# YIVEK/aom-av1-lavish

Measured on AMD Instinct MI355X. Metric: superblocks/s (fwd_txfm+quant+SAD RDO inner loop), 1080p cpu-used=6, 1/2/4/8 GPU, higher is better.
Workload: dtype int32; 1 GPU; rdo: 1920x1080 8-bit frame per step; C2 fwd_txfm2d + quantize_fp (qindex 128) of all 14 TX sizes <=32x32 x every valid TX type + C3 DIAMOND full-pel search of every 16x16 block x 7 refs (downsampled SAD, MV_COST_ENTROPY default nmv context, sadperbit 4, errorperbit 31, cost list, step_param 0; candidate rows from the references' tiled copy, rebuilt per step); 510 SB64/frame; parallelism=frame-per-rank x1, legs=C3 on a second stream beside C2 (C3 in at most 384 workgroups)

## Files before the change

### aom-av1-lavish_amd/csrc/txq.hip

```cpp
#include <atomic>

#include "txq_dev.h"

namespace lavish {

template <int LS>
__device__ __forceinline__ int32_t quant_rt(int32_t c, bool ac, int kind, int highbd,
                                            const QP& qp) {
  if (kind == LAVISH_QUANT_FP)
    return highbd ? quant_one<LS, LAVISH_QUANT_FP, true>(c, ac, qp)
                  : quant_one<LS, LAVISH_QUANT_FP, false>(c, ac, qp);
  return highbd ? quant_one<LS, LAVISH_QUANT_B, true>(c, ac, qp)
                : quant_one<LS, LAVISH_QUANT_B, false>(c, ac, qp);
}

constexpr int kFrameStreams = 3;
constexpr int kFanDefault = 3;

template <int W, int H>
__global__ __launch_bounds__(256, 2) void txq_plane_kernel(TxqArgs a) {
  __shared__ __attribute__((aligned(16))) char lds[TxqLds<W, H>::kBytes];
  txq_plane_body<W, H>(a, blockIdx.x, lds);
}

template <int CLS>
__global__ __launch_bounds__(256, 2) void txq_multi_kernel(TxqDispatch d, TxqArgs a0, TxqArgs a1,
                                                           TxqArgs a2, TxqArgs a3, TxqArgs a4,
                                                           TxqArgs a5, TxqArgs a6, TxqArgs a7,
                                                           TxqArgs a8) {
  __shared__ __attribute__((aligned(16))) char lds[class_lds(CLS)];
  txq_multi_body<CLS>(d, a0, a1, a2, a3, a4, a5, a6, a7, a8, blockIdx.x, lds);
}

template <int LS>
__global__ __launch_bounds__(256) void quant_kernel(const int32_t* coeff, int n,
                                                     const int16_t* scan, int kind,
                                                     int highbd, QP qp,
                                                     int32_t* qcoeff, int32_t* dqcoeff,
                                                     uint16_t* eob) {
  __shared__ int red[4];
  const size_t base = (size_t)blockIdx.x * n;
  const int tid = threadIdx.x;
  int last = 0;
  for (int i = tid; i < n; i += 256) {
    const int rc = scan[i];
    const int32_t c = coeff[base + rc];
    const int32_t q = quant_rt<LS>(c, rc != 0, kind, highbd, qp);
    qcoeff[base + rc] = q;
    const int32_t cs = c >> 31, m = (q ^ cs) - cs;
    const int32_t d = rc != 0 ? qp.dequant[1] : qp.dequant[0];
    const int32_t dm = (int32_t)((uint32_t)m * (uint32_t)d) >> LS;
    dqcoeff[base + rc] = (dm ^ cs) - cs;
    if (q != 0) last = max(last, i + 1);
  }
#pragma unroll
  for (int m = 1; m < 64; m <<= 1) last = max(last, __shfl_xor(last, m));
  if ((tid & 63) == 0) red[tid >> 6] = last;
  __syncthreads();
  if (tid == 0) eob[blockIdx.x] = (uint16_t)max(max(red[0], red[1]), max(red[2], red[3]));
}

static void build_chunks(TxqArgs& a, int nbg) {
  int cnt = 0, sz[16] = {}, ti[16][16];
  for (int vk = 0; vk < 4; ++vk) {
    int n = 0;
    for (int i = 0; i < a.ntypes; ++i)
      if (((kVtxPacked >> (2 * a.types[i])) & 3) == (uint32_t)vk) ti[cnt][n++] = i;
    if (n) sz[cnt++] = n;
  }
  while (nbg * cnt < 2048 && cnt < 16) {
    int big = 0;
    for (int g = 1; g < cnt; ++g)
      if (sz[g] > sz[big]) big = g;
    if (sz[big] < 2) break;
    const int keep = (sz[big] + 1) / 2;
    for (int i = keep; i < sz[big]; ++i) ti[cnt][i - keep] = ti[big][i];
    sz[cnt++] = sz[big] - keep;
    sz[big] = keep;
  }
  int o = 0;
  for (int g = 0; g < cnt; ++g) {
    a.chunk_off[g] = o;
    for (int i = 0; i < sz[g]; ++i) a.chunk_ti[o++] = ti[g][i];
  }
  a.chunk_off[cnt] = o;
  a.tgroups = cnt;
}

template <int W, int H>
static int plan_plane(TxqArgs& a) {
  constexpr int P = Tile<W, H>::P * 4;
  const int nbg = (a.nblocks + P - 1) / P;
  if (nbg == 0) return 0;
  build_chunks(a, nbg);
  return ((nbg + 7) / 8) * 8 * a.tgroups;
}

template <int W, int H>
static void launch_plane(TxqArgs a, hipStream_t s) {
  const int grid = plan_plane<W, H>(a);
  if (grid == 0) return;
  hipLaunchKernelGGL((txq_plane_kernel<W, H>), dim3(grid), dim3(256), 0, s, a);
  LAVISH_CHECK(hipGetLastError());
}

static int plan_size(int tx_size, TxqArgs& a) {
  switch (tx_size) {
    case 0: return plan_plane<4, 4>(a);
    case 1: return plan_plane<8, 8>(a);
    case 2: return plan_plane<16, 16>(a);
    case 3: return plan_plane<32, 32>(a);
    case 5: return plan_plane<4, 8>(a);
    case 6: return plan_plane<8, 4>(a);
    case 7: return plan_plane<8, 16>(a);
    case 8: return plan_plane<16, 8>(a);
    case 9: return plan_plane<16, 32>(a);
    case 10: return plan_plane<32, 16>(a);
    case 13: return plan_plane<4, 16>(a);
    case 14: return plan_plane<16, 4>(a);
    case 15: return plan_plane<8, 32>(a);
    case 16: return plan_plane<32, 8>(a);
    default: return -1;
  }
}

static QP to_qp(const LavishQuantParams* p) {
  QP q{};
  if (p) {
    for (int i = 0; i < 2; ++i) {
      q.zbin[i] = p->zbin[i];
      q.round[i] = p->round[i];
      q.quant[i] = p->quant[i];
      q.quant_shift[i] = p->quant_shift[i];
      q.dequant[i] = p->dequant[i];
    }
  }
  return q;
}

int txq_args(const int16_t* residual, int stride, int width, int height, int tx_size,
             uint32_t type_mask, int bd, int quant_kind, const LavishQuantParams* qp,
             int32_t* qcoeff, int32_t* dqcoeff, uint16_t* eob, int32_t* coeff, TxqArgs& a);

int txq_plane(const int16_t* residual, int stride, int width, int height, int tx_size,
              uint32_t type_mask, int bd, int quant_kind, const LavishQuantParams* qp,
              int32_t* qcoeff, int32_t* dqcoeff, uint16_t* eob, int32_t* coeff,
              hipStream_t s) {
  if (tx_size < 0 || tx_size >= 19) return -1;
  const int W = tx_w(tx_size), H = tx_h(tx_size);
  if (quant_kind < 0 || quant_kind > 2) return -3;
  if (quant_kind != LAVISH_QUANT_NONE && qp == nullptr) return -3;
  if (quant_kind == LAVISH_QUANT_FP && !quant_fp_params_ok(qp)) return kErrQuantParams;
  if (width <= 0 || height <= 0 || stride < width) return -4;
  if (W > 32 || H > 32)
    return txq_plane_64(residual, stride, width, height, tx_size, type_mask, bd, quant_kind, qp,
                        qcoeff, dqcoeff, eob, coeff, s);
  TxqArgs a{};
  const int rc = txq_args(residual, stride, width, height, tx_size, type_mask, bd, quant_kind,
                          qp, qcoeff, dqcoeff, eob, coeff, a);
  if (rc) return rc;
  switch (tx_size) {
    case 0: launch_plane<4, 4>(a, s); break;
    case 1: launch_plane<8, 8>(a, s); break;
    case 2: launch_plane<16, 16>(a, s); break;
    case 3: launch_plane<32, 32>(a, s); break;
    case 5: launch_plane<4, 8>(a, s); break;
    case 6: launch_plane<8, 4>(a, s); break;
    case 7: launch_plane<8, 16>(a, s); break;
    case 8: launch_plane<16, 8>(a, s); break;
    case 9: launch_plane<16, 32>(a, s); break;
    case 10: launch_plane<32, 16>(a, s); break;
    case 13: launch_plane<4, 16>(a, s); break;
    case 14: launch_plane<16, 4>(a, s); break;
    case 15: launch_plane<8, 32>(a, s); break;
    case 16: launch_plane<32, 8>(a, s); break;
    default: return -2;
  }
  return 0;
}

int txq_args(const int16_t* residual, int stride, int width, int height, int tx_size,
             uint32_t type_mask, int bd, int quant_kind, const LavishQuantParams* qp,
             int32_t* qcoeff, int32_t* dqcoeff, uint16_t* eob, int32_t* coeff, TxqArgs& a) {
  const int W = tx_w(tx_size), H = tx_h(tx_size);
// ... 30 lines not shown
    case 0:
      hipLaunchKernelGGL(quant_kernel<0>, dim3(nblocks), dim3(256), 0, s, coeff, n, scan,
                         quant_kind, hb, q, qcoeff, dqcoeff, eob);
      break;
    case 1:
      hipLaunchKernelGGL(quant_kernel<1>, dim3(nblocks), dim3(256), 0, s, coeff, n, scan,
                         quant_kind, hb, q, qcoeff, dqcoeff, eob);
      break;
    case 2:
      hipLaunchKernelGGL(quant_kernel<2>, dim3(nblocks), dim3(256), 0, s, coeff, n, scan,
                         quant_kind, hb, q, qcoeff, dqcoeff, eob);
      break;
    default:
      return -2;
  }
  LAVISH_CHECK(hipGetLastError());
  return 0;
}

struct FrameStreams {
  int device = -1;
  hipStream_t s[kFrameStreams] = {};
  hipEvent_t fork = nullptr, join[kFrameStreams] = {};
};
static thread_local FrameStreams t_fs;
struct FanSet {
  FrameStreams fs;
};
static thread_local FanSet* t_fan_own = nullptr;

static void frame_streams_init(FrameStreams& f, int dev) {
  for (int i = 1; i < kFrameStreams; ++i) {
    LAVISH_CHECK(hipStreamCreateWithFlags(&f.s[i], hipStreamNonBlocking));
    LAVISH_CHECK(hipEventCreateWithFlags(&f.join[i], hipEventDisableTiming));
  }
  LAVISH_CHECK(hipEventCreateWithFlags(&f.fork, hipEventDisableTiming));
  f.device = dev;
}

static FrameStreams& frame_streams() {
  if (t_fan_own != nullptr) return t_fan_own->fs;
  int dev = 0;
  LAVISH_CHECK(hipGetDevice(&dev));
  if (t_fs.device != dev) frame_streams_init(t_fs, dev);
  return t_fs;
}

FanSet* fan_create() {
  int dev = 0;
  LAVISH_CHECK(hipGetDevice(&dev));
  FanSet* f = new FanSet();
  frame_streams_init(f->fs, dev);
  return f;
}

void fan_destroy(FanSet* f) {
  if (f == nullptr) return;
  if (t_fan_own == f) t_fan_own = nullptr;
  for (int i = 1; i < kFrameStreams; ++i) {
    LAVISH_CHECK(hipStreamDestroy(f->fs.s[i]));
    LAVISH_CHECK(hipEventDestroy(f->fs.join[i]));
  }
  LAVISH_CHECK(hipEventDestroy(f->fs.fork));
  delete f;
}

void fan_use(FanSet* f) { t_fan_own = f; }

static std::atomic<int> g_fan_width{kFanDefault};
int fan_width() { return g_fan_width.load(std::memory_order_relaxed); }
int set_fan_width(int w) {
  if (w < 1 || w > kFrameStreams) return -1;
  g_fan_width.store(w, std::memory_order_relaxed);
  return 0;
}

hipStream_t* fan_out(hipStream_t caller) {
  FrameStreams& fs = frame_streams();
  fs.s[0] = caller;
  LAVISH_CHECK(hipEventRecord(fs.fork, caller));
  for (int i = 1; i < kFrameStreams; ++i) LAVISH_CHECK(hipStreamWaitEvent(fs.s[i], fs.fork, 0));
  return fs.s;
}

void fan_in(hipStream_t caller) {
  FrameStreams& fs = frame_streams();
  for (int i = 1; i < kFrameStreams; ++i) {
    LAVISH_CHECK(hipEventRecord(fs.join[i], fs.s[i]));
    LAVISH_CHECK(hipStreamWaitEvent(caller, fs.join[i], 0));
  }
}

int txq_frame_plan(const int16_t* residual, int stride, int width, int height, uint32_t size_mask,
                   const uint32_t* type_masks, int bd, int quant_kind, const LavishQuantParams* qp,
                   int32_t* const* qcoeff, int32_t* const* dqcoeff, uint16_t* const* eob, int cls,
                   TxqMulti& m, int& grid) {
  if (quant_kind == LAVISH_QUANT_FP && qp != nullptr && !quant_fp_params_ok(qp))
    return kErrQuantParams;
  int order[19], n = 0;
  for (int s = 0; s < 19; ++s)
    if (((size_mask >> s) & 1) && tx_w(s) <= 32 && tx_h(s) <= 32 && (txq_class(s) ? 1 : 0) == cls)
      order[n++] = s;
  auto work = [&](int s) {
    return (long)__builtin_popcount(type_masks[s]) * max_eob(s) * (width / tx_w(s)) *
           (height / tx_h(s));
  };
  for (int i = 1; i < n; ++i)
    for (int j = i; j > 0 && work(order[j]) > work(order[j - 1]); --j) {
      const int t = order[j];
      order[j] = order[j - 1];
      order[j - 1] = t;
    }
  m = TxqMulti{};
  int g = 0;
  for (int i = 0; i < n; ++i) {
    const int s = order[i];
    if (m.d.n == kMultiMax) return -2;
    TxqArgs& a = m.a[txq_slot(s)];
    const int rc = txq_args(residual, stride, width, height, s, type_masks[s], bd, quant_kind, qp,
                            qcoeff[s], dqcoeff[s], eob[s], nullptr, a);
    if (rc) return rc;
    const int sg = plan_size(s, a);
    if (sg <= 0) continue;
    m.d.code[m.d.n] = s;
    m.d.wg0[m.d.n] = g;
    g += sg;
    ++m.d.n;
  }
  m.d.wg0[m.d.n] = g;
  grid = g;
  return 0;
}

int txq_frame(const int16_t* residual, int stride, int width, int height, uint32_t size_mask,
              const uint32_t* type_masks, int bd, int quant_kind, const LavishQuantParams* qp,
              int32_t* const* qcoeff, int32_t* const* dqcoeff, uint16_t* const* eob,
              hipStream_t caller) {
  if (quant_kind == LAVISH_QUANT_FP && qp != nullptr && !quant_fp_params_ok(qp))
    return kErrQuantParams;
  for (int s = 0; s < 19; ++s) {
    if (!((size_mask >> s) & 1) || (tx_w(s) <= 32 && tx_h(s) <= 32)) continue;
    const int rc = txq_plane(residual, stride, width, height, s, type_masks[s], bd, quant_kind,
                             qp, qcoeff[s], dqcoeff[s], eob[s], nullptr, caller);
    if (rc) return rc;
  }
  for (int cls = 1; cls >= 0; --cls) {
    TxqMulti m;
    int g = 0;
    const int rc = txq_frame_plan(residual, stride, width, height, size_mask, type_masks, bd,
                                  quant_kind, qp, qcoeff, dqcoeff, eob, cls, m, g);
    if (rc) return rc;
    if (g == 0) continue;
    if (cls == 0)
      hipLaunchKernelGGL(txq_multi_kernel<0>, dim3(g), dim3(256), 0, caller, m.d, m.a[0], m.a[1],
                         m.a[2], m.a[3], m.a[4], m.a[5], m.a[6], m.a[7], m.a[8]);
    else
      hipLaunchKernelGGL(txq_multi_kernel<1>, dim3(g), dim3(256), 0, caller, m.d, m.a[0], m.a[1],
                         m.a[2], m.a[3], m.a[4], m.a[5], m.a[6], m.a[7], m.a[8]);
    LAVISH_CHECK(hipGetLastError());
  }
  return 0;
}

}

extern "C" int lavish_set_fan_width(int streams) { return lavish::set_fan_width(streams); }

extern "C" int lavish_txq_frame(const int16_t* residual, int stride, int width, int height,
                                uint32_t size_mask, const uint32_t* type_masks, int bit_depth,
                                int quant_kind, const LavishQuantParams* qp,
                                int32_t* const* qcoeff, int32_t* const* dqcoeff,
                                uint16_t* const* eob, void* stream) {
  return lavish::txq_frame(residual, stride, width, height, size_mask, type_masks, bit_depth,
                           quant_kind, qp, qcoeff, dqcoeff, eob, (hipStream_t)stream);
}

extern "C" int lavish_txq_plane(const int16_t* residual, int stride, int width, int height,
                                int tx_size, uint32_t type_mask, int bit_depth,
                                int quant_kind, const LavishQuantParams* qp,
                                int32_t* qcoeff, int32_t* dqcoeff, uint16_t* eob,
                                int32_t* coeff, void* stream) {
  return lavish::txq_plane(residual, stride, width, height, tx_size, type_mask, bit_depth,
                           quant_kind, qp, qcoeff, dqcoeff, eob, coeff,
                           (hipStream_t)stream);
}

extern "C" int lavish_quantize_batch(const int32_t* coeff, int n, int nblocks,
                                     const int16_t* scan, const int16_t* iscan,
                                     int log_scale, int bit_depth, int quant_kind,
                                     const LavishQuantParams* qp, int32_t* qcoeff,
                                     int32_t* dqcoeff, uint16_t* eob, void* stream) {
  (void)iscan;
  return lavish::quantize_batch(coeff, n, nblocks, scan, log_scale, bit_depth, quant_kind,
                                qp, qcoeff, dqcoeff, eob, (hipStream_t)stream);
}
```

### aom-av1-lavish_amd/csrc/txq_dev.h

```cpp
#pragma once

#include "lane_red.h"
#include "lavish_internal.h"
#include "quant_dev.h"

namespace lavish {

struct TxqArgs {
  const int16_t* res;
  int stride;
  int bw;
  int nblocks;
  int ntypes;
  int types[16];
  int tgroups;
  int chunk_off[17];
  int chunk_ti[16];
  int quant_kind;
  int highbd;
  QP qp;
  const int16_t* iscan_default;
  int32_t* qcoeff;
  int32_t* dqcoeff;
  uint16_t* eob;
  int32_t* coeff;
};

template <int W, int H>
struct Tile {
  static constexpr int MN = W < H ? W : H;
  static constexpr int P = 64 / MN;
  static constexpr int CPT = W / MN;
  static constexpr int RPT = H / MN;
  static constexpr int N = W * H;
  static constexpr int T1S = W + 1;
  static constexpr int T1 = P * H * T1S;
  static constexpr int T2 = P * N;
};

template <int W, int H, bool FAST, int QK, bool HBD>
__device__ __forceinline__ void txq_types(const TxqArgs& a,
                                          const int32_t (&res)[Tile<W, H>::CPT][H],
                                          int32_t* t1, int32_t* t2, const int16_t* isc, int lane,
                                          int blk0, int nvalid, int c0, int c1) {
  using C = TxCfg<W, H>;
  using T = Tile<W, H>;
  constexpr int N = T::N, T1S = T::T1S;
  constexpr int LS = C::log_scale;
  {
    const int t = __builtin_amdgcn_readfirstlane(a.types[a.chunk_ti[c0]]);
    const int vt = (kVtxPacked >> (2 * t)) & 3;
    const int kc = vt == 3 ? 2 : (vt == 0 ? 0 : 1);
    const bool ud = vt == 2;
#pragma unroll
    for (int k = 0; k < T::CPT; ++k) {
      const int j = k * 64 + lane;
      const int b = j / W, c = j % W;
      int32_t in[H], out[H];
#pragma unroll
      for (int r = 0; r < H; ++r) {
        const int32_t x = ud ? res[k][H - 1 - r] : res[k][r];
        if constexpr (FAST) in[r] = x * (1 << C::s0);
        else in[r] = round_shift_1<-C::s0>(x);
      }
      fwd_1d<H, C::cos_bit_col, FAST>(kc, in, out);
#pragma unroll
      for (int r = 0; r < H; ++r) t1[(b * H + r) * T1S + c] = round_shift_1<-C::s1>(out[r]);
    }
    wave_sync();
  }

  int qf_rnd[2], qf_thr1[2], qf_qt[2];
#pragma unroll
  for (int i = 0; i < 2; ++i) {
    qf_rnd[i] = (a.qp.round[i] + ((1 << LS) >> 1)) >> LS;
    qf_qt[i] = a.qp.quant[i];
    qf_thr1[i] = ((a.qp.dequant[i] + (1 << (1 + LS)) - 1) >> (1 + LS)) - 1;
  }

  for (int ci = c0; ci < c1; ++ci) {
    const int ti = __builtin_amdgcn_readfirstlane(a.chunk_ti[ci]);
    const int t = __builtin_amdgcn_readfirstlane(a.types[ti]);
    const int ht = (kHtxPacked >> (2 * t)) & 3;
    const int kr = ht == 3 ? 2 : (ht == 0 ? 0 : 1);
    const bool lr = ht == 2;
    const int skind = t < 10 ? 0 : ((t & 1) ? 1 : 2);

#pragma unroll
    for (int k = 0; k < T::RPT; ++k) {
      const int j = k * 64 + lane;
      const int b = j / H, r = j % H;
      int32_t in[W], out[W];
      const int32_t* row = t1 + (b * H + r) * T1S;
      if (lr) {
#pragma unroll
        for (int c = 0; c < W; ++c) in[c] = row[W - 1 - c];
      } else {
#pragma unroll
        for (int c = 0; c < W; ++c) in[c] = row[c];
      }
      fwd_1d<W, C::cos_bit_row, FAST>(kr, in, out);
      const size_t obase = ((size_t)ti * a.nblocks + blk0 + b) * N;
      const int16_t* iscan = isc + skind * N;
      int last = 0;
      if constexpr (QK == LAVISH_QUANT_FP && FAST && !HBD) {
        const bool dcl = r == 0;
        const int rnd0 = dcl ? qf_rnd[0] : qf_rnd[1];
        const int qt0 = dcl ? qf_qt[0] : qf_qt[1];
        const int thr0 = dcl ? qf_thr1[0] : qf_thr1[1];
#pragma unroll
        for (int c = 0; c < W; ++c) {
          int32_t v = round_shift_1<-C::s2>(out[c]);
          if constexpr (C::rect2) v = rshift64((int64_t)v * 5793, 12);
          const int rc = c * H + r;
          if (a.coeff != nullptr) {
            if (b < nvalid) a.coeff[obase + rc] = v;
          }
          const int32_t sgn = v >> 31;
          const int32_t av = (v ^ sgn) - sgn;
          const int32_t pass = ((c ? qf_thr1[1] : thr0) - av) >> 31;
          const int32_t t = min(av + (c ? qf_rnd[1] : rnd0), 32767);
          const int32_t qa = (mul_i24(t, c ? qf_qt[1] : qt0) >> (16 - LS)) & pass;
          const int32_t q = (qa ^ sgn) - sgn;
          t2[b * N + rc] = q;
          const int32_t nz = (qa + 0x7FFFFF) >> 23;
          last = max(last, ((int)iscan[rc] + 1) & -nz);
        }
      } else {
#pragma unroll
      for (int c = 0; c < W; ++c) {
        int32_t v = round_shift_1<-C::s2>(out[c]);
        if constexpr (C::rect2) v = rshift64((int64_t)v * 5793, 12);
        const int rc = c * H + r;
        int32_t q = 0;
        if constexpr (QK == LAVISH_QUANT_NONE) {
          if (b < nvalid) a.coeff[obase + rc] = v;
        } else {
          if (a.coeff != nullptr) {
            if (b < nvalid) a.coeff[obase + rc] = v;
          }
          q = quant_one<LS, QK, HBD, FAST>(v, c != 0 || r != 0, a.qp);
        }
        t2[b * N + rc] = q;
        const int pos1 = iscan[rc] + 1;
        last = q != 0 ? max(last, pos1) : last;
      }
      }
      last = lane_max<H>(last);
      if (r == 0 && b < nvalid && a.eob != nullptr)
        a.eob[(size_t)ti * a.nblocks + blk0 + b] = (uint16_t)last;
    }
    wave_sync();

    if (a.qcoeff != nullptr) {
      const int total = nvalid * N;
      const size_t gbase = ((size_t)ti * a.nblocks + blk0) * N;
      for (int i = lane * 4; i < total; i += 64 * 4) {
        const v4i q4 = *reinterpret_cast<const v4i*>(&t2[i]);
        __builtin_nontemporal_store(q4, reinterpret_cast<v4i*>(&a.qcoeff[gbase + i]));
        if (a.dqcoeff != nullptr) {
          const int rc0 = i % N;
          v4i d4;
          d4.x = dequant_one<LS, FAST>(q4.x, rc0 != 0, a.qp);
          d4.y = dequant_one<LS, FAST>(q4.y, 1, a.qp);
          d4.z = dequant_one<LS, FAST>(q4.z, 1, a.qp);
          d4.w = dequant_one<LS, FAST>(q4.w, 1, a.qp);
          __builtin_nontemporal_store(d4, reinterpret_cast<v4i*>(&a.dqcoeff[gbase + i]));
        }
      }
    }
    wave_sync();
  }
}

template <int W, int H>
struct TxqLds {
  using T = Tile<W, H>;
  static constexpr int kT2Off = (4 * T::T1 * 4 + 15) & ~15;
  static constexpr int kIscOff = kT2Off + 4 * T::T2 * 4;
  static constexpr int kBytes = kIscOff + 3 * T::N * 2;
};

template <int W, int H>
__device__ __forceinline__ void txq_plane_body(const TxqArgs& a, int id, char* lds) {
  using T = Tile<W, H>;
  using LL = TxqLds<W, H>;
  constexpr int H_ = H;
  int32_t* t1s = reinterpret_cast<int32_t*>(lds);
  int32_t* t2s = reinterpret_cast<int32_t*>(lds + LL::kT2Off);
  int16_t* isc = reinterpret_cast<int16_t*>(lds + LL::kIscOff);

  const int inner = id & 7, rest = id >> 3;
  const int tg = rest % a.tgroups, quad = (rest / a.tgroups) * 8 + inner;
  const int ntiles = (a.nblocks + T::P - 1) / T::P;
  if (quad * 4 >= ntiles) return;
  const int c0 = a.chunk_off[tg], c1 = a.chunk_off[tg + 1];

  const int tid = threadIdx.x;
  for (int i = tid; i < T::N; i += 256) {
    isc[i] = a.iscan_default[i];
    isc[T::N + i] = (int16_t)i;
    isc[2 * T::N + i] = (int16_t)((i % H) * W + i / H);
  }
  __syncthreads();

  const int wave = tid >> 6, lane = tid & 63;
  const int tile = quad * 4 + wave;
  if (tile >= ntiles) return;
  const int blk0 = tile * T::P;
  const int nvalid = min(T::P, a.nblocks - blk0);
  int32_t* t1 = t1s + wave * T::T1;
  int32_t* t2 = t2s + wave * T::T2;

  int32_t res[T::CPT][H_];
  int32_t amax = 0;
#pragma unroll
  for (int k = 0; k < T::CPT; ++k) {
    const int j = k * 64 + lane;
    const int b = j / W, c = j % W;
    const int blk = blk0 + b;
    if (b < nvalid) {
      const int by = blk / a.bw, bx = blk - by * a.bw;
      const int16_t* src = a.res + (size_t)by * H * a.stride + bx * W + c;
#pragma unroll
      for (int r = 0; r < H; ++r) {
        res[k][r] = src[(size_t)r * a.stride];
        amax = max(amax, abs(res[k][r]));
      }
    } else {
#pragma unroll
      for (int r = 0; r < H; ++r) res[k][r] = 0;
    }
  }
  const bool fast = __builtin_amdgcn_ballot_w64(amax > kFastResidualMax) == 0;
#define LAVISH_TXQ_RUN(F, Q, HB) \
  txq_types<W, H, F, Q, HB>(a, res, t1, t2, isc, lane, blk0, nvalid, c0, c1)
  const int qk = a.quant_kind;
  if (qk == LAVISH_QUANT_NONE) {
    if (fast) LAVISH_TXQ_RUN(true, LAVISH_QUANT_NONE, false);
    else LAVISH_TXQ_RUN(false, LAVISH_QUANT_NONE, false);
  } else if (qk == LAVISH_QUANT_FP) {
    if (a.highbd) {
      if (fast) LAVISH_TXQ_RUN(true, LAVISH_QUANT_FP, true);
      else LAVISH_TXQ_RUN(false, LAVISH_QUANT_FP, true);
    } else {
      if (fast) LAVISH_TXQ_RUN(true, LAVISH_QUANT_FP, false);
      else LAVISH_TXQ_RUN(false, LAVISH_QUANT_FP, false);
    }
  } else {
    if (a.highbd) {
      if (fast) LAVISH_TXQ_RUN(true, LAVISH_QUANT_B, true);
      else LAVISH_TXQ_RUN(false, LAVISH_QUANT_B, true);
    } else {
      if (fast) LAVISH_TXQ_RUN(true, LAVISH_QUANT_B, false);
      else LAVISH_TXQ_RUN(false, LAVISH_QUANT_B, false);
    }
  }
#undef LAVISH_TXQ_RUN
}

constexpr int kMultiMax = 9;
struct TxqDispatch {
  int code[kMultiMax];
  int wg0[kMultiMax + 1];
  int n;
};
struct TxqMulti {
  TxqArgs a[kMultiMax];
  TxqDispatch d;
};
__host__ __device__ constexpr int txq_slot(int s) {
  return s == 0 ? 0 : s == 1 ? 1 : s == 2 ? 2 : s == 5 ? 3 : s == 6 ? 4 : s == 7 ? 5
       : s == 8 ? 6 : s == 13 ? 7 : s == 14 ? 8
       : s == 3 ? 0 : s == 9 ? 1 : s == 10 ? 2 : s == 15 ? 3 : s == 16 ? 4 : -1;
}
static_assert(sizeof(TxqMulti) <= 4096, "kernel argument size");

constexpr int lds_bytes(int s) {
  return s == 0 ? TxqLds<4, 4>::kBytes : s == 1 ? TxqLds<8, 8>::kBytes
       : s == 2 ? TxqLds<16, 16>::kBytes : s == 3 ? TxqLds<32, 32>::kBytes
       : s == 5 ? TxqLds<4, 8>::kBytes : s == 6 ? TxqLds<8, 4>::kBytes
       : s == 7 ? TxqLds<8, 16>::kBytes : s == 8 ? TxqLds<16, 8>::kBytes
       : s == 9 ? TxqLds<16, 32>::kBytes : s == 10 ? TxqLds<32, 16>::kBytes
       : s == 13 ? TxqLds<4, 16>::kBytes : s == 14 ? TxqLds<16, 4>::kBytes
       : s == 15 ? TxqLds<8, 32>::kBytes : s == 16 ? TxqLds<32, 8>::kBytes : 0;
}
__host__ __device__ constexpr bool txq_class(int s) {
  return s == 3 || s == 9 || s == 10 || s == 15 || s == 16;
}
constexpr int class_lds(int cls) {
  int m = 16;
  for (int s = 0; s < 17; ++s)
    if ((s < 4 || s > 4) && s != 11 && s != 12 && lds_bytes(s) > 0 && (txq_class(s) ? 1 : 0) == cls)
      m = lds_bytes(s) > m ? lds_bytes(s) : m;
  return m;
}

template <int CLS>
__device__ __forceinline__ void txq_multi_body(const TxqDispatch& d, const TxqArgs& a0,
                                               const TxqArgs& a1, const TxqArgs& a2,
                                               const TxqArgs& a3, const TxqArgs& a4,
                                               const TxqArgs& a5, const TxqArgs& a6,
                                               const TxqArgs& a7, const TxqArgs& a8, int g,
                                               char* lds) {
  int code = d.code[0], id = g;
#pragma unroll
  for (int k = 1; k < kMultiMax; ++k) {
    if (k < d.n && g >= d.wg0[k]) {
      code = d.code[k];
      id = g - d.wg0[k];
    }
  }
  if constexpr (CLS == 0) {
    switch (code) {
      case 0: txq_plane_body<4, 4>(a0, id, lds); break;
      case 1: txq_plane_body<8, 8>(a1, id, lds); break;
      case 2: txq_plane_body<16, 16>(a2, id, lds); break;
      case 5: txq_plane_body<4, 8>(a3, id, lds); break;
      case 6: txq_plane_body<8, 4>(a4, id, lds); break;
      case 7: txq_plane_body<8, 16>(a5, id, lds); break;
      case 8: txq_plane_body<16, 8>(a6, id, lds); break;
      case 13: txq_plane_body<4, 16>(a7, id, lds); break;
      case 14: txq_plane_body<16, 4>(a8, id, lds); break;
      default: break;
    }
  } else {
    switch (code) {
      case 3: txq_plane_body<32, 32>(a0, id, lds); break;
      case 9: txq_plane_body<16, 32>(a1, id, lds); break;
      case 10: txq_plane_body<32, 16>(a2, id, lds); break;
      case 15: txq_plane_body<8, 32>(a3, id, lds); break;
      case 16: txq_plane_body<32, 8>(a4, id, lds); break;
      default: break;
    }
  }
}

int txq_frame_plan(const int16_t* residual, int stride, int width, int height, uint32_t size_mask,
                   const uint32_t* type_masks, int bd, int quant_kind, const LavishQuantParams* qp,
                   int32_t* const* qcoeff, int32_t* const* dqcoeff, uint16_t* const* eob, int cls,
                   TxqMulti& m, int& grid);

int txq_frame(const int16_t* residual, int stride, int width, int height, uint32_t size_mask,
              const uint32_t* type_masks, int bd, int quant_kind, const LavishQuantParams* qp,
              int32_t* const* qcoeff, int32_t* const* dqcoeff, uint16_t* const* eob,
              hipStream_t caller);

}
```

### aom-av1-lavish_amd/lavish_dsp/__init__.py

```python
import ctypes
import os

import numpy as np

_HERE = os.path.dirname(os.path.abspath(__file__))
LIB_PATH = os.environ.get("LAVISH_HIP_LIB") or os.path.join(os.path.dirname(_HERE),
                                                            "liblavish_hip.so")

if not os.path.exists(LIB_PATH):
    raise ImportError(
        "liblavish_hip.so not found at %s -- build it with `make -C aom-av1-lavish_amd` "
        "(or __graft_entry__.build()); there is no CPU fallback" % LIB_PATH)

try:
    import torch
except ImportError:
    pass

_lib = ctypes.CDLL(LIB_PATH)

TX_SIZES = ["4x4", "8x8", "16x16", "32x32", "64x64", "4x8", "8x4", "8x16", "16x8",
            "16x32", "32x16", "32x64", "64x32", "4x16", "16x4", "8x32", "32x8", "16x64",
            "64x16"]
TX_W = [4, 8, 16, 32, 64, 4, 8, 8, 16, 16, 32, 32, 64, 4, 16, 8, 32, 16, 64]
# ... 4 lines not shown
QUANT_FP, QUANT_B, QUANT_NONE = 0, 1, 2


def max_eob(tx_size):
    if tx_size in (17, 18):
        return 512
    if TX_W[tx_size] == 64 or TX_H[tx_size] == 64:
        return 1024
    return TX_W[tx_size] * TX_H[tx_size]


def tx_scale(tx_size):
    p = TX_W[tx_size] * TX_H[tx_size]
    return int(p > 256) + int(p > 1024)


def tx_type_valid(tx_size, tx_type):
    m = max(TX_W[tx_size], TX_H[tx_size])
    if m == 64:
        return tx_type == 0
    if m == 32:
        return tx_type in (0, 9)
    return 0 <= tx_type < 16


def valid_type_mask(tx_size):
    return sum(1 << t for t in range(16) if tx_type_valid(tx_size, t))


class TxfmParam(ctypes.Structure):
    _fields_ = [("tx_type", ctypes.c_uint8), ("tx_size", ctypes.c_uint8),
                ("lossless", ctypes.c_int), ("bd", ctypes.c_int), ("is_hbd", ctypes.c_int),
                ("tx_set_type", ctypes.c_uint8), ("eob", ctypes.c_int)]


class QuantParams(ctypes.Structure):
    _fields_ = [(n, ctypes.c_int16 * 2) for n in
                ("zbin", "round", "quant", "quant_shift", "dequant")]

    def as_dict(self):
        return {n: np.array(list(getattr(self, n)), np.int16) for n, _ in self._fields_}


_vp, _i32, _i64 = ctypes.c_void_p, ctypes.c_int, ctypes.c_int64
_lib.lavish_hip_status.restype = _i32
_lib.lavish_hip_status_string.restype = ctypes.c_char_p
_lib.lavish_hip_set_abort_on_error.argtypes = [_i32]
_lib.lavish_hip_init.argtypes = [_i32]
_lib.lavish_hip_version.restype = _i32
_lib.lavish_build_quant_params.argtypes = [_i32, _i32, _i32, _i32, _i32,
                                           ctypes.POINTER(QuantParams)]
_lib.lavish_scan.restype = ctypes.POINTER(ctypes.c_int16)
_lib.lavish_scan.argtypes = [_i32, _i32]
_lib.lavish_iscan.restype = ctypes.POINTER(ctypes.c_int16)
_lib.lavish_iscan.argtypes = [_i32, _i32]
_lib.lavish_txq_plane.argtypes = [_vp, _i32, _i32, _i32, _i32, ctypes.c_uint32, _i32, _i32,
                                  ctypes.POINTER(QuantParams), _vp, _vp, _vp, _vp, _vp]
_lib.lavish_txq_plane.restype = _i32
_lib.lavish_txq_frame.argtypes = [_vp, _i32, _i32, _i32, ctypes.c_uint32, _vp, _i32, _i32,
                                  ctypes.POINTER(QuantParams), _vp, _vp, _vp, _vp]
_lib.lavish_txq_frame.restype = _i32
_lib.lavish_quantize_batch.argtypes = [_vp, _i32, _i32, _vp, _vp, _i32, _i32, _i32,
                                       ctypes.POINTER(QuantParams), _vp, _vp, _vp, _vp]
_lib.lavish_quantize_batch.restype = _i32

_FWD2D = {}
for _s, _name in enumerate(TX_SIZES):
    f = getattr(_lib, "av1_fwd_txfm2d_%s_hip" % _name)
    f.argtypes = [_vp, _vp, _i32, ctypes.c_uint8, _i32]
    f.restype = None
    _FWD2D[_s] = f
_lib.av1_lowbd_fwd_txfm_hip.argtypes = [_vp, _vp, _i32, ctypes.POINTER(TxfmParam)]


class PlaneQuant(ctypes.Structure):
    _fields_ = [(n, ctypes.c_int16 * 2) for n in
                ("zbin", "round_fp", "quant_fp", "round", "quant", "quant_shift", "dequant")]


_lib.lavish_build_plane_quant.argtypes = [_i32, _i32, _i32, _i32, ctypes.POINTER(PlaneQuant)]
_lib.lavish_build_plane_quant.restype = _i32
_lib.lavish_av1_quant_batch.argtypes = [_vp, _i32, _i32, _i32, _i32, ctypes.POINTER(PlaneQuant),
                                        _i32, _i32, ctypes.c_uint32, _i32, _vp, _vp, _vp, _vp,
                                        _vp, _vp]
_lib.lavish_av1_quant_batch.restype = _i32
AV1_QUANT_FP, AV1_QUANT_B, AV1_QUANT_DC, AV1_QUANT_SKIP, AV1_QUANT_SATD_GATE = range(5)


def build_plane_quant(bit_depth, qindex, quant_sharpness=0, y_dc_delta_q=0):
    q = PlaneQuant()
    if _lib.lavish_build_plane_quant(bit_depth, qindex, quant_sharpness, y_dc_delta_q,
                                     ctypes.byref(q)) != 0:
        raise ValueError("lavish_build_plane_quant(%d, %d) failed" % (bit_depth, qindex))
    return q


def av1_quant_batch(coeff, tx_size, tx_type, bit_depth, pq, mode, skip_trellis=0,
                    threshold=0xFFFFFFFF, qstep=0, dc_only=None, stream=None):
    import torch
    n = max_eob(tx_size)
    assert coeff.dtype == torch.int32 and coeff.is_contiguous() and coeff.shape[-1] == n
    nb = coeff.numel() // n
    qc, dq = torch.empty_like(coeff), torch.empty_like(coeff)
    eob = torch.empty(nb, dtype=torch.int16, device=coeff.device)
    flags = torch.empty(nb, dtype=torch.uint8, device=coeff.device)
    if dc_only is not None:
        assert dc_only.dtype == torch.uint8 and dc_only.numel() >= nb and dc_only.is_cuda
    rc = _lib.lavish_av1_quant_batch(_p_t(coeff), nb, tx_size, tx_type, bit_depth,
                                     ctypes.byref(pq), mode, skip_trellis, threshold, qstep,
                                     _p_t(dc_only) if dc_only is not None else None, _p_t(qc),
                                     _p_t(dq), _p_t(eob), _p_t(flags), _stream_ptr(stream))
    if rc != 0:
        raise ValueError("lavish_av1_quant_batch rejected its arguments (rc=%d)" % rc)
    return qc, dq, eob, flags


def _p_t(t):
    return ctypes.c_void_p(t.data_ptr())


class BitDepthInfo(ctypes.Structure):
    _fields_ = [("bit_depth", ctypes.c_int), ("use_highbitdepth_buf", ctypes.c_int)]


_lib.av1_quick_txfm_hip.argtypes = [_i32, ctypes.c_uint8, BitDepthInfo, _vp, _i32, _vp]
_lib.av1_quick_txfm_hip.restype = None

_QARGS = [_vp, ctypes.c_ssize_t, _vp, _vp, _vp, _vp, _vp, _vp, _vp, _vp, _vp, _vp]
_QUANT_NAMES = ["av1_quantize_fp", "av1_quantize_fp_32x32", "av1_quantize_fp_64x64",
                "aom_quantize_b", "aom_quantize_b_32x32", "aom_quantize_b_64x64",
                "aom_highbd_quantize_b", "aom_highbd_quantize_b_32x32",
                "aom_highbd_quantize_b_64x64"]
for _n in _QUANT_NAMES:
    getattr(_lib, _n + "_hip").argtypes = _QARGS
_lib.av1_highbd_quantize_fp_hip.argtypes = _QARGS + [_i32]


def lib():
    return _lib


def status():
    return _lib.lavish_hip_status(), _lib.lavish_hip_status_string().decode()


_lib.lavish_set_fan_width.argtypes = [ctypes.c_int]
_lib.lavish_set_fan_width.restype = ctypes.c_int


def set_fan_width(streams):
    rc = _lib.lavish_set_fan_width(int(streams))
    if rc != 0:
        raise ValueError("lavish_set_fan_width(%r): %d" % (streams, rc))


def _p(a):
    return a.ctypes.data_as(ctypes.c_void_p)


def build_quant_params(bit_depth, qindex, kind=QUANT_FP, quant_sharpness=0, y_dc_delta_q=0):
    q = QuantParams()
    rc = _lib.lavish_build_quant_params(bit_depth, qindex, quant_sharpness, y_dc_delta_q,
                                        kind, ctypes.byref(q))
    if rc != 0:
        raise ValueError("lavish_build_quant_params(%d, %d) failed" % (bit_depth, qindex))
    return q


def scan_order(tx_size, tx_type):
    n = min(TX_W[tx_size], 32) * min(TX_H[tx_size], 32)
    s = np.ctypeslib.as_array(_lib.lavish_scan(tx_size, tx_type), shape=(n,)).copy()
    i = np.ctypeslib.as_array(_lib.lavish_iscan(tx_size, tx_type), shape=(n,)).copy()
    return s, i


def _fwd2d(tx_size):
    def fn(input, output, stride, tx_type, bd):
        assert input.dtype == np.int16 and output.dtype == np.int32
        assert input.size >= (TX_H[tx_size] - 1) * stride + TX_W[tx_size]
        assert output.size >= TX_W[tx_size] * TX_H[tx_size]
        _FWD2D[tx_size](_p(input), _p(output), stride, tx_type, bd)
    fn.__name__ = "av1_fwd_txfm2d_" + TX_SIZES[tx_size]
    return fn


for _s in _FWD2D:
    globals()["av1_fwd_txfm2d_" + TX_SIZES[_s]] = _fwd2d(_s)


def av1_lowbd_fwd_txfm(src_diff, coeff, diff_stride, txfm_param):
    _lib.av1_lowbd_fwd_txfm_hip(_p(src_diff), _p(coeff), diff_stride, ctypes.byref(txfm_param))


def av1_quick_txfm(use_hadamard, tx_size, bd_info, src_diff, src_stride, coeff):
    _lib.av1_quick_txfm_hip(int(use_hadamard), tx_size, bd_info, _p(src_diff), src_stride,
                            _p(coeff))


def _quant(name):
    cfn = getattr(_lib, name + "_hip")

    def fn(coeff_ptr, n_coeffs, zbin_ptr, round_ptr, quant_ptr, quant_shift_ptr, qcoeff_ptr,
           dqcoeff_ptr, dequant_ptr, eob_ptr, scan, iscan):
        cfn(_p(coeff_ptr), n_coeffs, _p(zbin_ptr), _p(round_ptr), _p(quant_ptr),
            _p(quant_shift_ptr), _p(qcoeff_ptr), _p(dqcoeff_ptr), _p(dequant_ptr), _p(eob_ptr),
            _p(scan), _p(iscan))
    fn.__name__ = name
    return fn


for _n in _QUANT_NAMES:
    globals()[_n] = _quant(_n)


def av1_highbd_quantize_fp(coeff_ptr, count, zbin_ptr, round_ptr, quant_ptr, quant_shift_ptr,
                           qcoeff_ptr, dqcoeff_ptr, dequant_ptr, eob_ptr, scan, iscan,
                           log_scale):
    _lib.av1_highbd_quantize_fp_hip(_p(coeff_ptr), count, _p(zbin_ptr), _p(round_ptr),
                                    _p(quant_ptr), _p(quant_shift_ptr), _p(qcoeff_ptr),
                                    _p(dqcoeff_ptr), _p(dequant_ptr), _p(eob_ptr), _p(scan),
                                    _p(iscan), log_scale)


def _stream_ptr(stream):
    import torch
    s = stream if stream is not None else torch.cuda.current_stream()
    return ctypes.c_void_p(s.cuda_stream)


def txq_plane_out(residual, tx_size, type_mask, with_coeff=False):
    import torch
    H, W = residual.shape
    nb = (W // TX_W[tx_size]) * (H // TX_H[tx_size])
    nt = bin(type_mask).count("1")
    n = max_eob(tx_size)
    dev = residual.device
    out = {
        "qcoeff": torch.empty((nt, nb, n), dtype=torch.int32, device=dev),
        "dqcoeff": torch.empty((nt, nb, n), dtype=torch.int32, device=dev),
        "eob": torch.empty((nt, nb), dtype=torch.int16, device=dev),
    }
    if with_coeff:
        out["coeff"] = torch.empty((nt, nb, n), dtype=torch.int32, device=dev)
    return out


def txq_plane(residual, tx_size, type_mask, qp, bit_depth=8, quant_kind=QUANT_FP, out=None,
              stride=None, width=None, height=None, with_coeff=False, stream=None):
    import torch
    assert residual.dtype == torch.int16 and residual.is_cuda
    assert residual.stride(1) == 1, "residual rows must be contiguous"
    if not 0 <= tx_size < len(TX_SIZES):
        raise ValueError("tx_size %d out of range" % tx_size)
    Hh, Ww = residual.shape
    stride = residual.stride(0) if stride is None else stride
    width = Ww if width is None else width
    height = Hh if height is None else height
    if out is None:
        out = txq_plane_out(residual[:height, :width], tx_size, type_mask, with_coeff)
    coeff = out.get("coeff")
    rc = _lib.lavish_txq_plane(
        ctypes.c_void_p(residual.data_ptr()), stride, width, height, tx_size, type_mask,
        bit_depth, quant_kind, ctypes.byref(qp) if qp is not None else None,
        ctypes.c_void_p(out["qcoeff"].data_ptr()), ctypes.c_void_p(out["dqcoeff"].data_ptr()),
        ctypes.c_void_p(out["eob"].data_ptr()),
        ctypes.c_void_p(coeff.data_ptr()) if coeff is not None else None, _stream_ptr(stream))
    if rc != 0:
        raise ValueError("lavish_txq_plane rejected arguments (rc=%d)" % rc)
    return out


class FrameOutputs:

    def __init__(self, residual, sizes, type_masks=None):
        self.sizes = list(sizes)
        self.type_masks = {s: (type_masks or {}).get(s, valid_type_mask(s)) for s in self.sizes}
        self.outs = {s: txq_plane_out(residual, s, self.type_masks[s]) for s in self.sizes}
        self.size_mask = sum(1 << s for s in self.sizes)
        P19 = ctypes.c_void_p * 19
        self.tm = (ctypes.c_uint32 * 19)(*[self.type_masks.get(s, 0) for s in range(19)])
        self.q = P19(*[self.outs[s]["qcoeff"].data_ptr() if s in self.outs else 0 for s in range(19)])
        self.dq = P19(*[self.outs[s]["dqcoeff"].data_ptr() if s in self.outs else 0 for s in range(19)])
        self.eob = P19(*[self.outs[s]["eob"].data_ptr() if s in self.outs else 0 for s in range(19)])


def txq_frame(residual, frame_out, qp, bit_depth=8, quant_kind=QUANT_FP, stream=None,
              size_mask=None):
    import torch
    assert residual.dtype == torch.int16 and residual.is_cuda
    assert residual.stride(1) == 1, "residual rows must be contiguous"
    H, W = residual.shape
    mask = frame_out.size_mask if size_mask is None else frame_out.size_mask & size_mask
    rc = _lib.lavish_txq_frame(ctypes.c_void_p(residual.data_ptr()), residual.stride(0), W, H,
                               mask, frame_out.tm, bit_depth, quant_kind,
                               ctypes.byref(qp), frame_out.q, frame_out.dq, frame_out.eob,
                               _stream_ptr(stream))
    if rc != 0:
        raise ValueError("lavish_txq_frame rejected arguments (rc=%d)" % rc)
    return frame_out.outs


def quantize_batch(coeff, scan, log_scale, qp, bit_depth=8, quant_kind=QUANT_FP, stream=None):
    import torch
    nb, n = coeff.shape
    q = torch.empty_like(coeff)
    dq = torch.empty_like(coeff)
# ... 293 lines not shown
```

### include/lavish_dsp.h

```cpp
#ifndef LAVISH_DSP_H_
#define LAVISH_DSP_H_

#include <stddef.h>
#include <stdint.h>

#ifdef __cplusplus
extern "C" {
#endif

int lavish_hip_status(void);
const char *lavish_hip_status_string(void);
void lavish_hip_set_abort_on_error(int on);
int lavish_hip_init(int device);
int lavish_hip_version(void);

typedef struct LavishTxfmParam {
  uint8_t tx_type;
  uint8_t tx_size;
  int lossless;
  int bd;
  int is_hbd;
  uint8_t tx_set_type;
  int eob;
} LavishTxfmParam;

typedef struct LavishQuantParams {
  int16_t zbin[2];
  int16_t round[2];
  int16_t quant[2];
  int16_t quant_shift[2];
  int16_t dequant[2];
} LavishQuantParams;

enum { LAVISH_QUANT_FP = 0, LAVISH_QUANT_B = 1, LAVISH_QUANT_NONE = 2 };

int lavish_build_quant_params(int bit_depth, int qindex, int quant_sharpness,
                              int y_dc_delta_q, int kind,
                              LavishQuantParams *out);

const int16_t *lavish_scan(int tx_size, int tx_type);
const int16_t *lavish_iscan(int tx_size, int tx_type);

int lavish_txq_plane(const int16_t *residual, int stride, int width,
                     int height, int tx_size, uint32_t type_mask,
                     int bit_depth, int quant_kind,
                     const LavishQuantParams *qp, int32_t *qcoeff,
                     int32_t *dqcoeff, uint16_t *eob, int32_t *coeff,
                     void *stream);

int lavish_set_fan_width(int streams);

int lavish_txq_frame(const int16_t *residual, int stride, int width,
                     int height, uint32_t size_mask,
                     const uint32_t *type_masks, int bit_depth,
                     int quant_kind, const LavishQuantParams *qp,
                     int32_t *const *qcoeff, int32_t *const *dqcoeff,
                     uint16_t *const *eob, void *stream);

int lavish_quantize_batch(const int32_t *coeff, int n, int nblocks,
                          const int16_t *scan, const int16_t *iscan,
                          int log_scale, int bit_depth, int quant_kind,
                          const LavishQuantParams *qp, int32_t *qcoeff,
                          int32_t *dqcoeff, uint16_t *eob, void *stream);

typedef struct LavishPlaneQuant {
  int16_t zbin[2], round_fp[2], quant_fp[2], round[2], quant[2], quant_shift[2],
      dequant[2];
} LavishPlaneQuant;
int lavish_build_plane_quant(int bit_depth, int qindex, int quant_sharpness,
                             int y_dc_delta_q, LavishPlaneQuant *out);

enum {
  LAVISH_AV1_QUANT_FP = 0,
  LAVISH_AV1_QUANT_B = 1,
  LAVISH_AV1_QUANT_DC = 2,
  LAVISH_AV1_QUANT_SKIP = 3,
  LAVISH_AV1_QUANT_SATD_GATE = 4
};

int lavish_av1_quant_batch(const int32_t *coeff, int nblocks, int tx_size,
                           int tx_type, int bit_depth, const LavishPlaneQuant *pq,
                           int mode, int skip_trellis,
                           unsigned coeff_opt_satd_threshold, int qstep,
                           const uint8_t *dc_only, int32_t *qcoeff, int32_t *dqcoeff,
                           uint16_t *eob, uint8_t *flags, void *stream);

int lavish_qm_level(int qindex, int first, int last);
int lavish_qm_table_offset(int tx_size);

int lavish_quantize_qm_batch(const int32_t *coeff, int n, int nblocks,
                             const int16_t *scan, const int16_t *iscan,
                             int log_scale, int bit_depth, int quant_kind,
                             const LavishQuantParams *qp, const uint8_t *qm,
                             const uint8_t *iqm, int32_t *qcoeff,
                             int32_t *dqcoeff, uint16_t *eob, void *stream);

int lavish_av1_quant_qm_batch(const int32_t *coeff, int nblocks, int tx_size,
                              int tx_type, int bit_depth,
                              const LavishPlaneQuant *pq, int mode,
                              int skip_trellis,
                              unsigned coeff_opt_satd_threshold, int qstep,
                              const uint8_t *dc_only, const uint8_t *qm,
                              const uint8_t *iqm, int dist_mode,
                              int32_t *qcoeff, int32_t *dqcoeff, uint16_t *eob,
                              uint8_t *flags, int64_t *dist, int64_t *sse,
                              void *stream);

int lavish_block_error_qm_batch(const int32_t *coeff, const int32_t *dqcoeff,
                                int n, int nblocks, const uint8_t *qmatrix,
                                const int16_t *scan, int64_t *err,
                                int64_t *ssz, void *stream);

typedef struct LavishCoeffCost {
  int32_t txb_skip_cost[13][2];
  int32_t base_eob_cost[4][3];
  int32_t base_cost[42][8];
  int32_t eob_extra_cost[9][2];
  int32_t dc_sign_cost[3][2];
  int32_t lps_cost[21][26];
} LavishCoeffCost;
typedef struct LavishEobCost {
  int32_t eob_cost[2][11];
} LavishEobCost;
typedef struct LavishCoeffCosts {
  LavishCoeffCost coeff_costs[5][2];
  LavishEobCost eob_costs[7][2];
} LavishCoeffCosts;
typedef struct LavishTxbCtx {
  int32_t txb_skip_ctx;
  int32_t dc_sign_ctx;
} LavishTxbCtx;

enum {
  LAVISH_COEFF_RATE_EXACT = 0,
  LAVISH_COEFF_RATE_LAPLACIAN = 1
};

int lavish_cost_coeffs_txb_batch(const LavishCoeffCosts *costs, const int32_t *qcoeff,
                                 const uint16_t *eob, int nblocks, int plane, int tx_size,
                                 int tx_type, const LavishTxbCtx *txb_ctx, int tx_type_cost,
                                 int mode, int32_t *rate, void *stream);

int lavish_optimize_b_batch(const LavishCoeffCosts *costs, const int32_t *tcoeff,
                            int32_t *qcoeff, int32_t *dqcoeff, uint16_t *eob, int nblocks,
                            int plane, int tx_size, int tx_type, int bit_depth, int is_inter,
                            int rdmult, int sharpness, const int16_t *dequant,
                            const LavishTxbCtx *txb_ctx, int tx_type_cost, int32_t *rate,
                            uint8_t *entropy_ctx, void *stream);

int lavish_optimize_b_qm_batch(const LavishCoeffCosts *costs, const int32_t *tcoeff,
                               int32_t *qcoeff, int32_t *dqcoeff, uint16_t *eob,
                               int nblocks, int plane, int tx_size, int tx_type,
                               int bit_depth, int is_inter, int rdmult, int sharpness,
                               const int16_t *dequant, const uint8_t *iqm,
                               const uint8_t *qm_dist, const LavishTxbCtx *txb_ctx,
                               int tx_type_cost, int32_t *rate, uint8_t *entropy_ctx,
                               void *stream);

typedef struct LavishPixJob {
  int64_t src_off;
  int64_t ref_off[4];
  int64_t aux_off;
  int32_t xoff, yoff;
} LavishPixJob;

int lavish_sad_batch(const void *src, int src_stride, const void *ref,
                     int ref_stride, int w, int h, const LavishPixJob *jobs,
                     int njobs, int nrefs, int mode, const void *second_pred,
                     int highbd, uint32_t *sad_out, void *stream);

int lavish_variance_batch(const void *a, int a_stride, const void *b,
                          int b_stride, int w, int h, const LavishPixJob *jobs,
                          int njobs, int kind, int bit_depth, int highbd,
                          const void *second_pred, uint32_t *var_out,
                          uint32_t *sse_out, int32_t *sum_out,
                          int64_t *sse64_out, void *stream);

int lavish_subtract_batch(int rows, int cols, int16_t *diff, int diff_stride,
                          const void *src, int src_stride, const void *pred,
                          int pred_stride, const LavishPixJob *jobs,
                          int njobs, int highbd, void *stream);

int lavish_sum_squares_batch(const int16_t *src, int stride, int w, int h,
                             const LavishPixJob *jobs, int njobs,
                             uint64_t *out, void *stream);

int lavish_hadamard_batch(int n, int highbd, const int16_t *src_diff,
                          int stride, const LavishPixJob *jobs, int njobs,
                          int32_t *coeff, void *stream);

int lavish_satd_batch(const int32_t *coeff, int length, int nblocks, int *out,
                      void *stream);

int lavish_block_error_batch(const int32_t *coeff, const int32_t *dqcoeff,
                             int n, int nblocks, int bit_depth, int64_t *err,
                             int64_t *ssz, void *stream);

int lavish_hadamard_lp_batch(int n, const int16_t *src_diff, int stride,
                             const LavishPixJob *jobs, int njobs,
                             int16_t *coeff, void *stream);
int lavish_satd_lp_batch(const int16_t *coeff, int length, int nblocks,
                         int *out, void *stream);
int lavish_block_error_lp_batch(const int16_t *coeff, const int16_t *dqcoeff,
// ... 1195 lines not shown
```

Before: 837,400 SB64/s.

## Stage residuals in LDS instead of registers and raise class-0 txq occupancy

The per-lane residual array held in registers is replaced by staging the loaded residual columns into the wave's t2 LDS region, and the first column transform reads them back from LDS. This frees VGPRs so the class-0 multi kernel can be specialized with amdgpu_waves_per_eu(5,5) and dynamic LDS, aiming at higher occupancy. The trade is extra LDS writes and reads per block and a tight register budget that could cause spills. A small helper exporting the class LDS size is also added.

Measured after the change: 852,200 SB64/s (median of 6 runs). +1.8%, better.

```diff
diff --git a/aom-av1-lavish_amd/csrc/txq.hip b/aom-av1-lavish_amd/csrc/txq.hip
--- a/aom-av1-lavish_amd/csrc/txq.hip
+++ b/aom-av1-lavish_amd/csrc/txq.hip
@@ -30,6 +30,14 @@
                                                            TxqArgs a8) {
   __shared__ __attribute__((aligned(16))) char lds[class_lds(CLS)];
   txq_multi_body<CLS>(d, a0, a1, a2, a3, a4, a5, a6, a7, a8, blockIdx.x, lds);
+}
+
+template <>
+__global__ __launch_bounds__(256) __attribute__((amdgpu_waves_per_eu(5, 5))) void
+txq_multi_kernel<0>(TxqDispatch d, TxqArgs a0, TxqArgs a1, TxqArgs a2, TxqArgs a3, TxqArgs a4,
+                    TxqArgs a5, TxqArgs a6, TxqArgs a7, TxqArgs a8) {
+  extern __shared__ __attribute__((aligned(16))) char dyn_lds[];
+  txq_multi_body<0>(d, a0, a1, a2, a3, a4, a5, a6, a7, a8, blockIdx.x, dyn_lds);
 }
 
 template <int LS>
@@ -366,8 +374,8 @@
     if (rc) return rc;
     if (g == 0) continue;
     if (cls == 0)
-      hipLaunchKernelGGL(txq_multi_kernel<0>, dim3(g), dim3(256), 0, caller, m.d, m.a[0], m.a[1],
-                         m.a[2], m.a[3], m.a[4], m.a[5], m.a[6], m.a[7], m.a[8]);
+      hipLaunchKernelGGL(txq_multi_kernel<0>, dim3(g), dim3(256), class_lds(0), caller, m.d,
+                         m.a[0], m.a[1], m.a[2], m.a[3], m.a[4], m.a[5], m.a[6], m.a[7], m.a[8]);
     else
       hipLaunchKernelGGL(txq_multi_kernel<1>, dim3(g), dim3(256), 0, caller, m.d, m.a[0], m.a[1],
                          m.a[2], m.a[3], m.a[4], m.a[5], m.a[6], m.a[7], m.a[8]);
@@ -379,6 +387,10 @@
 }
 
 extern "C" int lavish_set_fan_width(int streams) { return lavish::set_fan_width(streams); }
+
+extern "C" int lavish_txq_class_lds(int cls) {
+  return cls == 0 || cls == 1 ? lavish::class_lds(cls) : -1;
+}
 
 extern "C" int lavish_txq_frame(const int16_t* residual, int stride, int width, int height,
                                 uint32_t size_mask, const uint32_t* type_masks, int bit_depth,
diff --git a/aom-av1-lavish_amd/csrc/txq_dev.h b/aom-av1-lavish_amd/csrc/txq_dev.h
--- a/aom-av1-lavish_amd/csrc/txq_dev.h
+++ b/aom-av1-lavish_amd/csrc/txq_dev.h
@@ -39,10 +39,9 @@
 };
 
 template <int W, int H, bool FAST, int QK, bool HBD>
-__device__ __forceinline__ void txq_types(const TxqArgs& a,
-                                          const int32_t (&res)[Tile<W, H>::CPT][H],
-                                          int32_t* t1, int32_t* t2, const int16_t* isc, int lane,
-                                          int blk0, int nvalid, int c0, int c1) {
+__device__ __forceinline__ void txq_types(const TxqArgs& a, int32_t* t1, int32_t* t2,
+                                          const int16_t* isc, int lane, int blk0, int nvalid,
+                                          int c0, int c1) {
   using C = TxCfg<W, H>;
   using T = Tile<W, H>;
   constexpr int N = T::N, T1S = T::T1S;
@@ -57,11 +56,18 @@
       const int j = k * 64 + lane;
       const int b = j / W, c = j % W;
       int32_t in[H], out[H];
+      const int32_t* col = t2 + k * H * 64 + lane;
+      if (ud) {
+#pragma unroll
+        for (int r = 0; r < H; ++r) in[r] = col[(H - 1 - r) * 64];
+      } else {
+#pragma unroll
+        for (int r = 0; r < H; ++r) in[r] = col[r * 64];
+      }
 #pragma unroll
       for (int r = 0; r < H; ++r) {
-        const int32_t x = ud ? res[k][H - 1 - r] : res[k][r];
-        if constexpr (FAST) in[r] = x * (1 << C::s0);
-        else in[r] = round_shift_1<-C::s0>(x);
+        if constexpr (FAST) in[r] = in[r] * (1 << C::s0);
+        else in[r] = round_shift_1<-C::s0>(in[r]);
       }
       fwd_1d<H, C::cos_bit_col, FAST>(kc, in, out);
 #pragma unroll
@@ -204,15 +210,14 @@
   }
   __syncthreads();
 
-  const int wave = tid >> 6, lane = tid & 63;
+  const int wave = __builtin_amdgcn_readfirstlane(tid >> 6), lane = tid & 63;
   const int tile = quad * 4 + wave;
   if (tile >= ntiles) return;
   const int blk0 = tile * T::P;
   const int nvalid = min(T::P, a.nblocks - blk0);
   int32_t* t1 = t1s + wave * T::T1;
-  int32_t* t2 = t2s + wave * T::T2;
-
-  int32_t res[T::CPT][H_];
+  int32_t* stage = t2s + wave * T::T2;
+
   int32_t amax = 0;
 #pragma unroll
   for (int k = 0; k < T::CPT; ++k) {
@@ -224,17 +229,21 @@
       const int16_t* src = a.res + (size_t)by * H * a.stride + bx * W + c;
 #pragma unroll
       for (int r = 0; r < H; ++r) {
-        res[k][r] = src[(size_t)r * a.stride];
-        amax = max(amax, abs(res[k][r]));
+        const int32_t x = src[(size_t)r * a.stride];
+        stage[(k * H_ + r) * 64 + lane] = x;
+        amax = max(amax, abs(x));
       }
     } else {
 #pragma unroll
-      for (int r = 0; r < H; ++r) res[k][r] = 0;
-    }
-  }
+      for (int r = 0; r < H; ++r) stage[(k * H_ + r) * 64 + lane] = 0;
+    }
+  }
+  int wave2 = wave;
+  asm volatile("" : "+s"(wave2));
+  int32_t* t2 = t2s + wave2 * T::T2;
   const bool fast = __builtin_amdgcn_ballot_w64(amax > kFastResidualMax) == 0;
 #define LAVISH_TXQ_RUN(F, Q, HB) \
-  txq_types<W, H, F, Q, HB>(a, res, t1, t2, isc, lane, blk0, nvalid, c0, c1)
+  txq_types<W, H, F, Q, HB>(a, t1, t2, isc, lane, blk0, nvalid, c0, c1)
   const int qk = a.quant_kind;
   if (qk == LAVISH_QUANT_NONE) {
     if (fast) LAVISH_TXQ_RUN(true, LAVISH_QUANT_NONE, false);
diff --git a/aom-av1-lavish_amd/lavish_dsp/__init__.py b/aom-av1-lavish_amd/lavish_dsp/__init__.py
--- a/aom-av1-lavish_amd/lavish_dsp/__init__.py
+++ b/aom-av1-lavish_amd/lavish_dsp/__init__.py
@@ -180,6 +180,15 @@
     rc = _lib.lavish_set_fan_width(int(streams))
     if rc != 0:
         raise ValueError("lavish_set_fan_width(%r): %d" % (streams, rc))
+
+
+def txq_class_lds(cls):
+    fn = _lib.lavish_txq_class_lds
+    fn.argtypes, fn.restype = [ctypes.c_int], ctypes.c_int
+    n = fn(int(cls))
+    if n < 0:
+        raise ValueError("lavish_txq_class_lds(%r): %d" % (cls, n))
+    return n
 
 
 def _p(a):
diff --git a/include/lavish_dsp.h b/include/lavish_dsp.h
--- a/include/lavish_dsp.h
+++ b/include/lavish_dsp.h
@@ -49,6 +49,8 @@
                      void *stream);
 
 int lavish_set_fan_width(int streams);
+
+int lavish_txq_class_lds(int cls);
 
 int lavish_txq_frame(const int16_t *residual, int stride, int width,
                      int height, uint32_t size_mask,
```
